# helgeanl/GP-MPC

Measured on NVIDIA H100. Metric: GP predictions/sec (N train x horizon test, fp64), higher is better.
Workload: dtype f64

## Files before the change

gp-mpc_b200/csrc/gpmpc.cu:

```cuda
#include "../../include/gpmpc.h"

#include <dlfcn.h>
#include <math.h>
#include <stdarg.h>
#include <stdlib.h>
#include <string.h>

#include <algorithm>
#include <array>
#include <functional>
#include <map>
#include <memory>
#include <type_traits>
#include <vector>

#include <nvtx3/nvToolsExt.h>

#include "common.cuh"
#include "gemm_dmma.cuh"
#include "predict_streamk.cuh"
#include "kernels.cuh"

#define GPMPC_VERSION 100
#define HB 64
// ... 1060 lines not shown
    if (!strcmp(name, "nlml_batch_max")) {
        if (!(value >= 0.0 && value <= 1e9)) { set_error(h, "nlml_batch_max must be >= 0"); return GPMPC_ERR_ARG; }
        h->opt_nlml_batch_max = (int)value; return GPMPC_OK;
    }
    set_error(h, "unknown option %s", name);
    return GPMPC_ERR_ARG;
}

static inline int ks_chunk(gpmpc_handle_t h)
{
    if (h->Npad < 8192) return 128;
    return (h->nloc >= 2 && h->Nx <= 12) ? 1024 : 512;
}

static inline int ks_blocks(gpmpc_handle_t h) { return (h->Npad + ks_chunk(h) - 1) / ks_chunk(h); }

static inline int round8(int n) { return (n + 7) / 8 * 8; }

static int ensure_rows(gpmpc_handle_t h)
{
    ENSURE(h->dV, (long long)h->nloc * HB * h->Npad);
    ENSURE(h->dR, (long long)h->nloc * HB * h->Npad);
    return GPMPC_OK;
}

static int ensure_predict_bufs(gpmpc_handle_t h, int H)
{
    const long long np = h->Npad, nt = np / 128;
    ENSURE(h->dKST, (long long)h->nloc * HB * np);
    ENSURE(h->dPMJ, (long long)h->nloc * HB * ks_blocks(h) * (h->Nx + 1));
    ENSURE(h->dSQ, (long long)h->nloc * HB * nt);
    ENSURE(h->dCnt, (long long)h->nloc * nt + h->nloc + 1);
    ENSURE(h->dPart, (long long)std::max(h->psk_ctas, h->opt_predict_ctas) * 2 * HB * PSK_BN);
    if (h->opt_refine) {
        int rc = ensure_rows(h);
        if (rc) return rc;
        ENSURE(h->dR2, (long long)h->nloc * HB * np);
    }
    if (H > h->Hcap) {
        h->Hcap = 0;
        h->dZ = h->dSigma = h->dMean = h->dVar = h->dJ = h->dCov = nullptr;
        const long long cap = std::max(H, HB);
        const int nyp = h->nloc_max * h->world;
        const long long Nx = h->Nx, Ny = h->Ny;
        ENSURE(h->dG, (long long)nyp * cap * (Nx + 2));
        ENSURE(h->dIn, cap * Nx + cap * Nx * Nx);
        ENSURE(h->dOut, cap * (2 * Ny + Ny * Nx + Ny * Ny));
        h->dZ = h->dIn; h->dSigma = h->dIn + cap * Nx;
        h->dMean = h->dOut; h->dVar = h->dOut + cap * Ny; h->dJ = h->dOut + 2 * cap * Ny;
        h->dCov = h->dOut + 2 * cap * Ny + cap * Ny * Nx;
        h->Hcap = (int)cap;
    }
    return GPMPC_OK;
}

template <int BM>
static cudaError_t psk_launch_bm(const PredictParams& p, const double* A, long long sA, const double* B, long long sB,
                                 int np, int grid, cudaStream_t st)
{
    constexpr int BYTES = psk_pipe_doubles(BM) * 8 + 2 * PSK_STAGES * 8 + 1024;
    const cudaError_t e = smem_opt_in<predict_streamk_kernel<BM>>(BYTES);
    if (e != cudaSuccess) return e;
    CUtensorMap tmA, tmB;
    if (!tmap_make(&tmA, A, np, BM, np, sA, p.nloc, BM)) return cudaErrorInvalidValue;
    if (!tmap_make(&tmB, B, np, np, np, sB, p.nloc, PSK_BN)) return cudaErrorInvalidValue;
    cudaLaunchConfig_t cfg;
    memset(&cfg, 0, sizeof(cfg));
    cfg.gridDim = dim3(grid); cfg.blockDim = dim3(PSK_THREADS); cfg.dynamicSmemBytes = BYTES; cfg.stream = st;
    cudaLaunchAttribute attr[1];
    attr[0].id = cudaLaunchAttributeProgrammaticStreamSerialization;
    attr[0].val.programmaticStreamSerializationAllowed = 1;
    cfg.attrs = attr; cfg.numAttrs = 1;
    return cudaLaunchKernelEx(&cfg, predict_streamk_kernel<BM>, p, tmA, tmB);
}

static int psk_grid(gpmpc_handle_t h, long long G)
{
    int ctas = h->opt_predict_ctas > 0 ? h->opt_predict_ctas : h->psk_ctas;
    ctas = std::min(ctas, PSK_MAX_CTAS);
    const long long by_work = std::max(1LL, G / 4);
    return (int)std::min<long long>(ctas, h->opt_predict_ctas > 0 ? G : by_work);
}

static cudaError_t psk_launch(gpmpc_handle_t h, const PredictParams& p0, const double* A, const double* B)
{
    const long long sA = (long long)HB * h->Npad, sB = slab(h);
    const int np = h->Npad, grid = psk_grid(h, p0.G);
    PredictParams p = p0;
    if (B == h->dLi.p && !p.upper) {
        for (int a = 0; a < h->nloc; ++a)
            if (h->panel_row[a] < np) return cudaErrorIllegalState;
        p.Lp = h->dLiP;
    }
    switch (round8(p.Hc)) {
    case 8: return psk_launch_bm<8>(p, A, sA, B, sB, np, grid, h->st);
    case 16: return psk_launch_bm<16>(p, A, sA, B, sB, np, grid, h->st);
    case 24: return psk_launch_bm<24>(p, A, sA, B, sB, np, grid, h->st);
    case 32: return psk_launch_bm<32>(p, A, sA, B, sB, np, grid, h->st);
    case 40: return psk_launch_bm<40>(p, A, sA, B, sB, np, grid, h->st);
    case 48: return psk_launch_bm<48>(p, A, sA, B, sB, np, grid, h->st);
    case 56: return psk_launch_bm<56>(p, A, sA, B, sB, np, grid, h->st);
    default: return psk_launch_bm<64>(p, A, sA, B, sB, np, grid, h->st);
    }
}

static void psk_base(gpmpc_handle_t h, PredictParams& p, int Hc, int upper = 0)
{
    memset(&p, 0, sizeof(p));
    const long long nt = h->Npad / 128;
    p.nloc = h->nloc; p.nt = (int)nt; p.Hc = Hc; p.upper = upper;
    p.ntb = (int)((h->Npad + PSK_BN - 1) / PSK_BN); p.nk = h->Npad / GEMM_BK;
    p.T = psk_steps_per_output(p.ntb, p.nk, upper); p.G = p.T * h->nloc;
    p.part = h->dPart;
    p.tile_cnt = h->dCnt; p.out_cnt = h->dCnt + (long long)h->nloc * nt; p.done_cnt = p.out_cnt + h->nloc;
    p.SQ = h->dSQ;
    p.hyp = h->dHyp; p.hyp_ld = h->Nx + 2; p.Nx = h->Nx;
}

static int panel_refresh(gpmpc_handle_t h)
{
    PredictParams p;
    psk_base(h, p, HB);
    const long long blk = PSK_BN * GEMM_BK;
    const double* old = h->dLiP;
    ENSURE(h->dLiP, p.G * blk);
    if (h->dLiP.p != old) panel_stale(h, -1, 0);
    for (int a = 0; a < h->nloc; ++a) {
        if (h->panel_row[a] >= h->Npad) continue;
        const int jt0 = h->panel_row[a] / PSK_BN;
        panel_pack_kernel<<<dim3(p.nk, p.ntb - jt0), 256, 0, h->st>>>(h->dLi + a * slab(h), h->Npad, h->dLiP + a * p.T * blk,
                                                                      p.ntb, jt0);
        CUDA_TRY(cudaGetLastError());
        h->panel_row[a] = h->Npad;
    }
    return GPMPC_OK;
}

static void psk_finalize(gpmpc_handle_t h, PredictParams& p, int H, int h0)
{
    p.finalize = 1; p.PMJ = h->dPMJ; p.nblk_mj = ks_blocks(h);
    p.Gloc = h->dG; p.slot0 = h->a0; p.Htot = H; p.h0 = h0;
}

static AssembleArgs assemble_args(gpmpc_handle_t h, int H, int method, const double* Sigma, int spp,
                                  double* mean, double* var, double* J, double* cov)
{
    AssembleArgs as;
    memset(&as, 0, sizeof(as));
    as.G = h->dG; as.Ny = h->Ny; as.Nx = h->Nx; as.H = H; as.method_ta = (method == GPMPC_METHOD_TA);
    as.Sigma = Sigma; as.sigma_per_point = spp;
    as.mean = mean; as.var = var; as.J = J; as.cov = cov;
    as.world = 1;
    as.stage_g = (assemble_rows_doubles(H, h->Ny, h->Nx) <= psk_pipe_doubles(round8(std::min(H, HB)))) ? 1 : 0;
    return as;
}

template <int NXP, int CH>
static cudaError_t launch_ks(gpmpc_handle_t h, const double* dZc, int Hc)
{
    const int smem = (NXP + 1) * CH * 8, nblk = ks_blocks(h);
    const cudaError_t e = smem_opt_in<ks_tile_kernel<NXP, CH>>(smem);
    if (e != cudaSuccess) return e;
    dim3 g(nblk, round8(Hc) / 8, h->nloc);
    ks_tile_kernel<NXP, CH><<<g, 256, smem, h->st>>>(h->dXT, h->Npad, h->N, h->Nx, h->dHyp, h->Nx + 2, h->dAlpha, h->Npad,
                                                     dZc, Hc, h->dKST, h->Npad, (long long)HB * h->Npad, h->dPMJ, nblk);
    return cudaGetLastError();
}

template <int CH>
static cudaError_t launch_ks_nx(gpmpc_handle_t h, const double* dZc, int Hc)
{
    const int Nx = h->Nx;
    if (Nx <= 4) return launch_ks<4, CH>(h, dZc, Hc);
    if (Nx <= 6) return launch_ks<6, CH>(h, dZc, Hc);
    if (Nx <= 8) return launch_ks<8, CH>(h, dZc, Hc);
    if (Nx <= 10) return launch_ks<10, CH>(h, dZc, Hc);
// ... 1658 lines not shown
    }
    if (world > 1) {
        if (!nccl_load(h->err, sizeof(h->err))) return GPMPC_ERR_NCCL;
        nccl_uid_t id;
        memcpy(&id, id128, 128);
        int r = g_nccl.CommInitRank(&h->comm, world, id, rank);
        if (r) { set_error(h, "ncclCommInitRank failed: %s", g_nccl.GetErrorString ? g_nccl.GetErrorString(r) : "?"); return GPMPC_ERR_NCCL; }
    }
    h->rank = rank; h->world = world; h->nloc_max = nlm;
    h->Hcap = 0;
    return GPMPC_OK;
}

extern "C" int gpmpc_peer_export(gpmpc_handle_t h, int Hcap, void* handle64)
{
    if (!h || !handle64 || Hcap < 1) return GPMPC_ERR_ARG;
    CUDA_TRY(cudaSetDevice(h->device));
    if (h->world > GPMPC_MAXW) { set_error(h, "peer exchange supports at most %d ranks", GPMPC_MAXW); return GPMPC_ERR_ARG; }
    if (h->dPeerBlock) { set_error(h, "gpmpc_peer_export: already exported"); return GPMPC_ERR_STATE; }
    const int nyp = h->nloc_max * h->world;
    h->peerGsz = (long long)nyp * Hcap * (h->Nx + 2);
    h->peerHcap = Hcap;
    ENSURE(h->dPeerBlock, 2 * GPMPC_MAXW + 2 * h->peerGsz);
    if (!h->dPeerStatus) {
        CUDA_TRY(cudaHostAlloc((void**)&h->hPeerStatus, sizeof(int), cudaHostAllocMapped));
        *h->hPeerStatus = 0;
        CUDA_TRY(cudaHostGetDevicePointer((void**)&h->dPeerStatus, h->hPeerStatus, 0));
    }
    CUDA_TRY(cudaStreamSynchronize(h->st));
    cudaIpcMemHandle_t mh;
    CUDA_TRY(cudaIpcGetMemHandle(&mh, h->dPeerBlock));
    static_assert(sizeof(cudaIpcMemHandle_t) == 64, "IPC handle size");
    memcpy(handle64, &mh, 64);
    return GPMPC_OK;
}

extern "C" int gpmpc_peer_attach(gpmpc_handle_t h, const void* handles)
{
    if (!h || !handles) return GPMPC_ERR_ARG;
    if (!h->dPeerBlock) { set_error(h, "gpmpc_peer_attach: call gpmpc_peer_export first"); return GPMPC_ERR_STATE; }
    CUDA_TRY(cudaSetDevice(h->device));
    for (int r = 0; r < h->world; ++r) {
        if (r == h->rank) { h->peerBase[r] = h->dPeerBlock; continue; }
        cudaIpcMemHandle_t mh;
        memcpy(&mh, (const char*)handles + 64 * r, 64);
        void* ptr = nullptr;
        CUDA_TRY(cudaIpcOpenMemHandle(&ptr, mh, cudaIpcMemLazyEnablePeerAccess));
        h->peerBase[r] = (double*)ptr; h->peerOpened[r] = true;
    }
    h->peer_ready = true; h->peer_step = 0;
    return GPMPC_OK;
}

extern "C" int gpmpc_get_size(gpmpc_handle_t h, int* N, int* Nx, int* Ny)
{
    if (!h) return GPMPC_ERR_ARG;
    if (N) *N = h->N;
    if (Nx) *Nx = h->Nx;
    if (Ny) *Ny = h->Ny;
    return GPMPC_OK;
}

extern "C" void* gpmpc_stream(gpmpc_handle_t h) { return h ? (void*)h->st : nullptr; }

extern "C" int gpmpc_synchronize(gpmpc_handle_t h)
{
    if (!h) return GPMPC_ERR_ARG;
    CUDA_TRY(cudaSetDevice(h->device));
    CUDA_TRY(cudaStreamSynchronize(h->st));
    return peer_status_check(h);
}

template <typename Setup>
static int profile_product(gpmpc_handle_t h, const char* fn, int H, const double* out, bool all_outputs, int n_tail,
                           Setup&& setup, std::vector<unsigned long long>& t, int* grid)
{
    if (!h || !out || H < 1 || H > HB) return GPMPC_ERR_ARG;
    int rc = predict_guard(h, fn, GPMPC_METHOD_TA, H);
    if (rc) return rc;
    rc = predict_prepare(h, fn, HB, all_outputs);
    if (rc) return rc;
    PredictParams p;
    psk_base(h, p, H);
    *grid = psk_grid(h, p.G);
    DevBuf<unsigned long long> dbg;
    ENSURE(dbg, (long long)*grid * 2 + n_tail);
    p.dbg = dbg;
    setup(p, dbg + 2 * *grid);
    for (int rep = 0; rep < 2; ++rep) {
        const cudaError_t e = psk_launch(h, p, h->dKST, h->dLi);
        if (e != cudaSuccess) { set_error(h, "%s: %s", fn, cudaGetErrorString(e)); return GPMPC_ERR_CUDA; }
    }
    t.resize((size_t)*grid * 2 + n_tail);
    cudaMemcpyAsync(t.data(), dbg, t.size() * 8, cudaMemcpyDeviceToHost, h->st);
    cudaStreamSynchronize(h->st);
    return GPMPC_OK;
}

extern "C" int gpmpc_profile_balance(gpmpc_handle_t h, int H, double* out4)
{
    std::vector<unsigned long long> t; int grid = 0;
    const int rc = profile_product(h, __func__, H, out4, false, 0, [](PredictParams&, unsigned long long*) {}, t, &grid);
    if (rc) return rc;
    unsigned long long lo = ~0ull, hi = 0; double mn = 1e300, mx = 0.0, sum = 0.0;
    for (int c = 0; c < grid; ++c) {
        const double d = (double)(t[2 * c + 1] - t[2 * c]) * 1e-3;
        mn = std::min(mn, d); mx = std::max(mx, d); sum += d;
        lo = std::min(lo, t[2 * c]); hi = std::max(hi, t[2 * c + 1]);
    }
    out4[0] = mn; out4[1] = mx; out4[2] = sum / grid; out4[3] = (double)(hi - lo) * 1e-3;
    return GPMPC_OK;
}

extern "C" int gpmpc_profile_tail(gpmpc_handle_t h, int H, double* out8)
{
    std::vector<unsigned long long> t; int grid = 0;
    auto setup = [&](PredictParams& p, unsigned long long* tail) {
        psk_finalize(h, p, H, 0);
        p.as = assemble_args(h, H, GPMPC_METHOD_TA, h->dSigma, 0, h->dMean, h->dVar, h->dJ, h->dCov);
        p.as.dbg = tail;
        p.do_assemble = 1;
    };
    const int rc = profile_product(h, __func__, H, out8, true, 8, setup, t, &grid);
    if (rc) return rc;
    unsigned long long lo = ~0ull, hi = 0, hi2 = 0; int cmax = 0;
    for (int c = 0; c < grid; ++c) {
        lo = std::min(lo, t[2 * c]);
        if (t[2 * c + 1] > hi) { hi2 = hi; hi = t[2 * c + 1]; cmax = c; } else hi2 = std::max(hi2, t[2 * c + 1]);
    }
    for (int k = 0; k < 6; ++k) out8[k] = ((double)t[2 * grid + k] - (double)hi2) * 1e-3;
    out8[6] = (double)(hi - lo) * 1e-3;
    out8[7] = (double)(t[2 * cmax + 1] - t[2 * cmax]) * 1e-3;
    return GPMPC_OK;
}

extern "C" int gpmpc_profile_leaf(gpmpc_handle_t h, double* out15)
{
    if (!h || !out15) return GPMPC_ERR_ARG;
    int rc = model_guard(h, __func__, NEED_HYPER);
    if (rc) return rc;
    DevBuf<long long> d;
    ENSURE(d, 16);
    CUDA_TRY(cudaMemcpyToSymbol(d_leaf_prof, &d.p, sizeof(d.p)));
    for (int rep = 0; rep < 2 && rc == GPMPC_OK; ++rep) {
        rc = launch_kbuild(h, h->dHyp, h->dJit, h->dL, 1, 0);
        if (rc == GPMPC_OK) rc = potrf_inv_rec(h, h->dL, h->dLi, slab(h), slab(h), h->dInfo, 0, 128, 1, 1, h->dW1, h->dW2);
    }
    cudaStreamSynchronize(h->st);
    long long hst[16];
    cudaMemcpy(hst, d, sizeof(hst), cudaMemcpyDeviceToHost);
    long long* nul = nullptr;
    cudaMemcpyToSymbol(d_leaf_prof, &nul, sizeof(nul));
    for (int k = 0; k < 15; ++k) out15[k] = (double)(hst[k] - hst[0]);
    factor_stale(h);
    return rc;
}

extern "C" int gpmpc_profile(gpmpc_handle_t h, int what, int n, int reps, double* ms_out)
{
    if (!h || !ms_out || reps < 1) return GPMPC_ERR_ARG;
    int rc = model_guard(h, __func__, NEED_HYPER);
    if (rc) return rc;
    const int np = h->Npad, Hc = (n > 0 && n <= HB) ? n : 56;
    float ms = 0.f;
    auto run = [&]() -> int {
        switch (what) {
        case GPMPC_PROF_KBUILD_FULL: return launch_kbuild(h, h->dHyp, h->dJit, h->dL, 1, 1);
// ... 62 lines not shown
```

gp-mpc_b200/csrc/predict_streamk.cuh:

```cuda
#pragma once
#include "common.cuh"
#include "gemm_dmma.cuh"

#define GPMPC_MAXW 16
#define PSK_CW 8
#define PSK_BN (32 * PSK_CW)
#define PSK_STAGES 5
#define PSK_CTAS_PER_SM 1
#define PSK_THREADS (32 * PSK_CW)

__host__ __device__ constexpr long long psk_pipe_doubles(int bm) { return (long long)PSK_STAGES * (bm + PSK_BN) * GEMM_BK; }


struct PeerArgs {
    double* base[GPMPC_MAXW];
    int world, rank;
    long long goff;
    int flag_idx;
    unsigned long long step;
    long long timeout_clocks;
};

struct AssembleArgs {
    const double* G;
    int Ny, Nx, H, method_ta;
    const double* Sigma; int sigma_per_point;
    double *mean, *var, *J, *cov;
    const unsigned long long* flags;
    int world; unsigned long long step; int* status;
    long long timeout_clocks;
    unsigned long long* dbg;
    int stage_g;
};

struct PredictParams {
    int nloc, nt, Hc;
    int ntb, nk;
    int upper;
    const double* Lp;
    long long T, G;
    double* part;
    unsigned int* tile_cnt;
    unsigned int* out_cnt;
    unsigned int* done_cnt;
    double* SQ;
    double* Vout; long long sV; int ldv;
    int finalize;
    const double* PMJ; int nblk_mj;
    const double* hyp; int hyp_ld, Nx;
    double* Gloc; int slot0, Htot, h0;
    PeerArgs pa; int use_peers, publish;
    AssembleArgs as; int do_assemble;
    unsigned long long* dbg;
};

__device__ __forceinline__ void tail_stamp(unsigned long long* dbg, int k, int tid)
{
    if (dbg && tid == 0) { unsigned long long t; asm volatile("mov.u64 %0, %%globaltimer;" : "=l"(t)); dbg[k] = t; }
}

template <bool WARP>
__device__ __forceinline__ void assemble_point(const AssembleArgs& A, int h, double* sh, int tid, int nth)
{
    const int Ny = A.Ny, Nx = A.Nx, H = A.H;
    double* Jh = sh; double* JS = sh + Ny * Nx; double* vh = sh + 2 * Ny * Nx;
    for (int idx = tid; idx < Ny * Nx; idx += nth) {
        const int a = idx / Nx, d = idx % Nx;
        const double v = __ldcg(A.G + (((long long)a) * H + h) * (Nx + 2) + 2 + d);
        Jh[idx] = v;
        if (A.J) A.J[((long long)h * Ny + a) * Nx + d] = v;
    }
    for (int a = tid; a < Ny; a += nth) {
        const double* g = A.G + (((long long)a) * H + h) * (Nx + 2);
        const double m = __ldcg(g), v = __ldcg(g + 1);
        if (A.mean) A.mean[(long long)h * Ny + a] = m;
        if (A.var) A.var[(long long)h * Ny + a] = v;
        vh[a] = v;
    }
    if (WARP) __syncwarp(); else __syncthreads();
    if (A.cov) {
        if (A.method_ta) {
            const double* Sg = A.Sigma + (A.sigma_per_point ? (long long)h * Nx * Nx : 0);
            for (int idx = tid; idx < Ny * Nx; idx += nth) {
                const int a = idx / Nx, e = idx % Nx;
                double s = 0.0;
                for (int d = 0; d < Nx; ++d) s = fma(Jh[a * Nx + d], Sg[d * Nx + e], s);
                JS[idx] = s;
            }
            if (WARP) __syncwarp(); else __syncthreads();
        }
        for (int idx = tid; idx < Ny * Ny; idx += nth) {
            const int a = idx / Ny, b = idx % Ny;
            double s = (a == b) ? vh[a] : 0.0;
            if (A.method_ta) {
                double t = 0.0;
                for (int e = 0; e < Nx; ++e) t = fma(JS[a * Nx + e], Jh[b * Nx + e], t);
                s += t;
            }
            A.cov[((long long)h * Ny + a) * Ny + b] = s;
        }
    }
    if (WARP) __syncwarp(); else __syncthreads();
}

__device__ __forceinline__ void assemble_flat_global(const AssembleArgs& A, double* JS, int tid, int nth)
{
    const int Ny = A.Ny, Nx = A.Nx, H = A.H, NyNx = Ny * Nx;
    const bool ta = A.cov && A.method_ta;
    for (int idx = tid; idx < H * NyNx; idx += nth) {
        const int h = idx / NyNx, r = idx - h * NyNx, a = r / Nx, e = r - a * Nx;
        const double* g = A.G + (((long long)a) * H + h) * (Nx + 2) + 2;
        if (A.J) A.J[idx] = __ldcg(g + e);
        if (ta) {
            const double* Sg = A.Sigma + (A.sigma_per_point ? (long long)h * Nx * Nx : 0);
            double s = 0.0;
            for (int d = 0; d < Nx; ++d) s = fma(__ldcg(g + d), Sg[d * Nx + e], s);
            JS[idx] = s;
        }
    }
    for (int idx = tid; idx < H * Ny; idx += nth) {
        const int h = idx / Ny, a = idx - h * Ny;
        const double* g = A.G + (((long long)a) * H + h) * (Nx + 2);
        if (A.mean) A.mean[idx] = __ldcg(g);
// ... 77 lines not shown
        const bool via_smem = Ny <= 8 && Ny <= NP;
        for (int idx = tid; idx < R; idx += nth) {
            const int h = idx / Ny, a = idx - h * Ny;
            const double var = Gs[idx * FP + 1];
            for (int b0 = 0; b0 < Ny; b0 += 8) {
                double acc[8];
#pragma unroll
                for (int k = 0; k < 8; ++k) acc[k] = 0.0;
                if (ta) {
                    for (int e = 0; e < Nx; ++e) {
                        const double je = JS[idx * NP + e];
#pragma unroll
                        for (int k = 0; k < 8; ++k) if (b0 + k < Ny) acc[k] = fma(je, Gs[(h * Ny + b0 + k) * FP + 2 + e], acc[k]);
                    }
                }
#pragma unroll
                for (int k = 0; k < 8; ++k) {
                    if (b0 + k < Ny) {
                        const double c = ((a == b0 + k) ? var : 0.0) + acc[k];
                        if (via_smem) JS[idx * NP + k] = c; else A.cov[(long long)idx * Ny + b0 + k] = c;
                    }
                }
            }
        }
        if (via_smem) {
            __syncthreads();
            for (int i = tid; i < R * Ny; i += nth) { const int row = i / Ny; A.cov[i] = JS[row * NP + (i - row * Ny)]; }
        }
    }
}

__device__ __forceinline__ void assemble_flat(const AssembleArgs& A, double* sh, int tid, int nth)
{
    if (A.stage_g) assemble_rows(A, sh, tid, nth);
    else assemble_flat_global(A, sh, tid, nth);
}

__device__ __forceinline__ bool peer_acquire(const AssembleArgs& A, int tid, int* sh_ok)
{
    if (!A.flags) return true;
    if (tid == 0) *sh_ok = 1;
    __syncthreads();
    if (tid < A.world) {
        const long long t0 = clock64();
        unsigned long long v;
        do {
            asm volatile("ld.acquire.sys.global.u64 %0, [%1];" : "=l"(v) : "l"(A.flags + tid) : "memory");
            if (v >= A.step) break;
            if (clock64() - t0 > A.timeout_clocks) {
                *reinterpret_cast<volatile int*>(A.status) = 1 + tid;
                *reinterpret_cast<volatile int*>(sh_ok) = 0;
                break;
            }
            __nanosleep(64);
        } while (true);
    }
    __syncthreads();
    return *reinterpret_cast<volatile int*>(sh_ok) != 0;
}

__global__ void __launch_bounds__(128)
assemble_kernel(const AssembleArgs A)
{
    extern __shared__ double sh[];
    __shared__ int ok;
    if (!peer_acquire(A, threadIdx.x, &ok)) return;
    for (int h = blockIdx.x; h < A.H; h += gridDim.x) assemble_point<false>(A, h, sh, threadIdx.x, blockDim.x);
}

#define PSK_SB (PSK_BN / GEMM_BK)
__host__ __device__ inline long long psk_kstart(int ntb, int nk, int upper, int jt)
{
    const long long full = (long long)(PSK_SB / 2) * jt * (jt + 1), d = (long long)PSK_SB * ntb - nk;
    return upper ? full - jt * d : (jt == ntb ? full - d : full);
}
__host__ __device__ inline long long psk_steps_per_output(int ntb, int nk, int upper) { return psk_kstart(ntb, nk, upper, ntb); }
__device__ __forceinline__ long long psk_kstart(const PredictParams& p, int jt) { return psk_kstart(p.ntb, p.nk, p.upper, jt); }
__host__ __device__ inline int psk_ksteps(int ntb, int nk, int upper, int jt)
{
    return upper ? nk - PSK_SB * (ntb - 1 - jt) : (PSK_SB * (jt + 1) < nk ? PSK_SB * (jt + 1) : nk);
}
__device__ __forceinline__ int psk_ksteps(const PredictParams& p, int jt) { return psk_ksteps(p.ntb, p.nk, p.upper, jt); }

struct PskIter { int a, jt, s, ks; };

__device__ __forceinline__ void psk_iter_init(PskIter& it, long long g, const PredictParams& p)
{
    it.a = (int)(g / p.T);
    const long long r = g - (long long)it.a * p.T;
    int jt = (int)((sqrt(8.0 * (double)r / PSK_SB + 1.0) - 1.0) * 0.5);
    jt = max(0, min(jt, p.ntb - 1));
    while (jt > 0 && psk_kstart(p, jt) > r) --jt;
    while (jt + 1 < p.ntb && psk_kstart(p, jt + 1) <= r) ++jt;
    it.jt = jt; it.s = (int)(r - psk_kstart(p, jt)); it.ks = psk_ksteps(p, jt);
}
__device__ __forceinline__ void psk_iter_next(PskIter& it, const PredictParams& p)
{
    if (++it.s == it.ks) {
        it.s = 0;
        if (++it.jt == p.ntb) { it.jt = 0; ++it.a; }
        it.ks = psk_ksteps(p, it.jt);
    }
}

__host__ __device__ inline long long psk_panel_chunk(int ntb, int nk, int jt, int s, int r, int c)
{
    return (psk_kstart(ntb, nk, 0, jt) + s) * (PSK_BN * GEMM_BK) + r * GEMM_BK + 2 * (c ^ (r & 7));
}

__global__ void __launch_bounds__(256)
panel_pack_kernel(const double* __restrict__ Li, int np, double* __restrict__ P, int ntb, int jt0)
{
    const int s = blockIdx.x, jt = jt0 + blockIdx.y, nk = np / GEMM_BK, c = threadIdx.x & 7;
    if (s >= psk_ksteps(ntb, nk, 0, jt)) return;
#pragma unroll 4
    for (int r = threadIdx.x >> 3; r < PSK_BN; r += 32) {
        const long long row = (long long)jt * PSK_BN + r;
        const double2 v = row < np ? __ldcs(reinterpret_cast<const double2*>(Li + row * np + s * GEMM_BK) + c) : make_double2(0.0, 0.0);
        *reinterpret_cast<double2*>(P + psk_panel_chunk(ntb, nk, jt, s, r, c)) = v;
    }
}

__device__ __forceinline__ void psk_store_record(const PredictParams& p, int a, int h, int q, double val)
{
    const long long off = (((long long)(p.slot0 + a)) * p.Htot + p.h0 + h) * (p.Nx + 2) + q;
    if (!p.use_peers) p.Gloc[off] = val;
    else for (int r = 0; r < p.pa.world; ++r) p.pa.base[r][p.pa.goff + off] = val;
}

__device__ __forceinline__ void psk_reduce_mj(const PredictParams& p, int i_begin, int i_end, int t, int nthr)
{
    const int F1 = p.Nx + 1;
    for (int i = i_begin + t; i < i_end; i += nthr) {
        const int ah = i / F1, qq = i - ah * F1, a = ah / p.Hc, h = ah - a * p.Hc;
        const double* pm = p.PMJ + ((long long)ah * p.nblk_mj) * F1 + qq;
        double s0 = 0.0, s1 = 0.0;
        int b = 0;
        for (; b + 16 <= p.nblk_mj; b += 16) {
            double v[16];
#pragma unroll
            for (int k = 0; k < 16; ++k) v[k] = __ldcg(pm + (long long)(b + k) * F1);
#pragma unroll
            for (int k = 0; k < 16; k += 2) { s0 += v[k]; s1 += v[k + 1]; }
        }
        for (; b + 2 <= p.nblk_mj; b += 2) { s0 += __ldcg(pm + (long long)b * F1); s1 += __ldcg(pm + (long long)(b + 1) * F1); }
        if (b < p.nblk_mj) s0 += __ldcg(pm + (long long)b * F1);
        psk_store_record(p, a, h, qq == 0 ? 0 : qq + 1, s0 + s1);
    }
}

__device__ __forceinline__ void psk_finalize_output(const PredictParams& p, int a, int tid, int nth)
{
    const int Nx = p.Nx;
    const double sf = p.hyp[(long long)a * p.hyp_ld + Nx];
    for (int base = 0; base < p.Hc; base += nth / 4) {
        const int h = base + (tid >> 2), j0 = tid & 3;
        double sj = 0.0;
        if (h < p.Hc) {
            const double* sq = p.SQ + ((long long)a * 64 + h) * p.nt;
            int j = j0;
            for (; j + 4 * 15 < p.nt; j += 4 * 16) {
                double v[16];
#pragma unroll
                for (int k = 0; k < 16; ++k) v[k] = __ldcg(sq + j + 4 * k);
#pragma unroll
                for (int k = 0; k < 16; ++k) sj += v[k];
            }
            for (; j < p.nt; j += 4) sj += __ldcg(sq + j);
        }
        sj += __shfl_xor_sync(0xffffffffu, sj, 1);
        sj += __shfl_xor_sync(0xffffffffu, sj, 2);
        if (h < p.Hc && j0 == 0) psk_store_record(p, a, h, 1, sf * sf - sj);
    }
    if (p.use_peers) __threadfence_system(); else __threadfence();
}

__device__ __forceinline__ void psk_step_tail(const PredictParams& p, double* sh, int tid, int nth,
                                              unsigned int* s_flag, int* s_ok)
{
    __syncthreads();
    if (tid == 0) {
        const unsigned int old = atomicAdd(p.done_cnt, 1u);
        const unsigned int last = (old == (unsigned int)(p.nloc - 1)) ? 1u : 0u;
        if (last) *p.done_cnt = 0u;
        *s_flag = last;
    }
    __syncthreads();
    if (*s_flag == 0u) return;
    if (p.finalize && p.use_peers && p.publish && tid == 0) {
        __threadfence_system();
        for (int r = 0; r < p.pa.world; ++r) {
            unsigned long long* f = reinterpret_cast<unsigned long long*>(p.pa.base[r]) + p.pa.flag_idx;
            asm volatile("st.release.sys.global.u64 [%0], %1;" :: "l"(f), "l"(p.pa.step) : "memory");
        }
    }
    tail_stamp(p.as.dbg, 2, tid);
    if (p.do_assemble) {
        __threadfence();
        if (peer_acquire(p.as, tid, s_ok)) assemble_flat(p.as, sh, tid, nth);
    }
    __syncthreads();
    tail_stamp(p.as.dbg, 5, tid);
}

__global__ void __launch_bounds__(128)
sq_rows_kernel(const double* __restrict__ V, int ldv, long long sV, double* __restrict__ SQ, int nt)
{
    __shared__ double red[4];
    const int jt = blockIdx.x, h = blockIdx.y, a = blockIdx.z;
    const double v = V[(long long)a * sV + (long long)h * ldv + jt * 128 + threadIdx.x];
    const double s = warp_sum(v * v);
    if ((threadIdx.x & 31) == 0) red[threadIdx.x >> 5] = s;
    __syncthreads();
    if (threadIdx.x == 0) SQ[((long long)a * 64 + h) * nt + jt] = (red[0] + red[1]) + (red[2] + red[3]);
}

__global__ void __launch_bounds__(PSK_THREADS)
finalize_kernel(const PredictParams p)
{
    extern __shared__ double sh[];
    __shared__ unsigned int s_flag;
    __shared__ int s_ok;
    const int per = p.Hc * (p.Nx + 1);
    psk_reduce_mj(p, blockIdx.x * per, (blockIdx.x + 1) * per, threadIdx.x, PSK_THREADS);
    psk_finalize_output(p, blockIdx.x, threadIdx.x, PSK_THREADS);
    psk_step_tail(p, sh, threadIdx.x, PSK_THREADS, &s_flag, &s_ok);
}

template <int BM>
__global__ void __launch_bounds__(PSK_THREADS, PSK_CTAS_PER_SM)
predict_streamk_kernel(const PredictParams p, const __grid_constant__ CUtensorMap tmA, const __grid_constant__ CUtensorMap tmB)
{
    constexpr int BK = GEMM_BK, BN = PSK_BN, STAGES = PSK_STAGES, CW = PSK_CW, NT = PSK_THREADS;
    constexpr int NF = BM / 8;
    static_assert(BK == 16 && BN == 32 * CW && BN % 128 == 0, "one m16n8k16 per fragment and k-step, 32 L-rows per warp");
    constexpr int GR = BN / 128;
    constexpr int A_STAGE = BM * BK, B_STAGE = BN * BK;
    constexpr uint32_t STAGE_TX = (BM + BN) * BK * 8;
    static_assert(BM % 8 == 0 && BM >= 8 && BM <= 64, "BM");

    extern __shared__ __align__(16) double smem_raw[];
    double* smem = smem_align1024(smem_raw);
    double* As = smem;
    double* Bs = smem + STAGES * A_STAGE;
    uint64_t* full = reinterpret_cast<uint64_t*>(smem + STAGES * (A_STAGE + B_STAGE));
    uint64_t* empty = full + STAGES;
    __shared__ double red[BN / 16][64];
    __shared__ unsigned int s_flag;
    __shared__ int s_ok;

    const int tid = threadIdx.x, warp = tid >> 5, lane = tid & 31, g = lane >> 2, t = lane & 3;
    const long long C = gridDim.x, c = blockIdx.x;
    const long long g0 = p.G * c / C;
    const int nsteps = (int)(p.G * (c + 1) / C - g0);
    if (nsteps <= 0) return;
    if (p.dbg && threadIdx.x == 0) { unsigned long long t0; asm volatile("mov.u64 %0, %%globaltimer;" : "=l"(t0)); p.dbg[2 * blockIdx.x] = t0; }

    __shared__ PskIter s_pit;
    __shared__ int s_pg;
    __shared__ uint64_t s_pol[2];
    __shared__ const double* s_lp;
    if (tid == 0) {
#pragma unroll
        for (int s = 0; s < STAGES; ++s) { mbar_init(full + s, 1); mbar_init(empty + s, CW); }
        mbar_fence_init();
    }
    __syncthreads();

    auto issue = [&]() {
        PskIter it = s_pit;
        const int pg = s_pg, s = pg % STAGES;
        if (pg >= STAGES) mbar_wait(empty + s, (uint32_t)(((pg / STAGES) - 1) & 1));
        mbar_arrive_expect_tx(full + s, STAGE_TX);
        const int jta = p.upper ? p.ntb - 1 - it.jt : it.jt;
        const int k0 = (p.upper ? jta * BN : 0) + it.s * BK;
        tma_tile_g2s_3d_hint(As + s * A_STAGE, &tmA, k0, 0, it.a, full + s, s_pol[1]);
        if (s_lp) bulk_g2s_hint(Bs + s * B_STAGE, s_lp + (long long)pg * B_STAGE, B_STAGE * 8, full + s, s_pol[0]);
        else tma_tile_g2s_3d_hint(Bs + s * B_STAGE, &tmB, k0, jta * BN, it.a, full + s, s_pol[0]);
        psk_iter_next(it, p);
        s_pit = it;
        s_pg = pg + 1;
    };
    constexpr int AHEAD = STAGES - 2;
    asm volatile("griddepcontrol.wait;" ::: "memory");
    if (tid == 0) {
        PskIter it;
        psk_iter_init(it, g0, p);
        s_pit = it; s_pg = 0;
        s_lp = p.Lp ? p.Lp + g0 * B_STAGE : nullptr;
        s_pol[0] = l2_policy_evict_first(); s_pol[1] = l2_policy_evict_last();
#pragma unroll
        for (int s = 0; s < AHEAD; ++s)
            if (s_pg < nsteps) issue();
    }
    if (p.finalize) {
        const int tot = p.nloc * p.Hc * (p.Nx + 1), per = (tot + (int)C - 1) / (int)C;
        if (tid >= 32) {
            psk_reduce_mj(p, min(tot, (int)c * per), min(tot, ((int)c + 1) * per), tid - 32, NT - 32);
            if (p.use_peers) __threadfence_system();
        }
    }

    PskIter cit;
    psk_iter_init(cit, g0, p);
    int cj[4];
#pragma unroll
    for (int j = 0; j < 4; ++j) cj[j] = (((j + 4 * (t >> 1)) ^ g) << 1) + (t & 1);
    int i = 0;
    while (i < nsteps) {
        const int a = cit.a, jt = cit.jt, s_begin = cit.s, ksteps = cit.ks;
        const int seg = min(ksteps - s_begin, nsteps - i);
        const int hh = warp / (128 / 32);
        const int st_lo = p.upper ? (128 / BK) * hh : 0;
        const int st_hi = p.upper ? ksteps : PSK_SB * jt + (128 / BK) * (hh + 1);
        double acc[2][NF][4];
#pragma unroll
        for (int mi = 0; mi < 2; ++mi)
#pragma unroll
            for (int ni = 0; ni < NF; ++ni)
#pragma unroll
                for (int r = 0; r < 4; ++r) acc[mi][ni][r] = 0.0;

        for (int q = 0; q < seg; ++q, ++i) {
            const int s = i % STAGES;
            if (tid == 0 && i + AHEAD < nsteps) issue();
            mbar_wait(full + s, (uint32_t)((i / STAGES) & 1));
            const int st = s_begin + q;
            if (st >= st_lo && st < st_hi) {
                const double* ls = Bs + s * B_STAGE + (warp * 32 + g) * 16;
                const double* ps = As + s * A_STAGE + g * 16;
                double av[2][8];
#pragma unroll
                for (int mi = 0; mi < 2; ++mi)
#pragma unroll
                    for (int j = 0; j < 4; ++j) { av[mi][2 * j] = ls[256 * mi + cj[j]]; av[mi][2 * j + 1] = ls[256 * mi + 128 + cj[j]]; }
#pragma unroll
                for (int ni = 0; ni < NF; ++ni) {
                    double bv[4];
#pragma unroll
                    for (int j = 0; j < 4; ++j) bv[j] = ps[ni * 8 * 16 + cj[j]];
                    dmma16816(acc[0][ni], av[0], bv);
                    dmma16816(acc[1][ni], av[1], bv);
                }
            }
            __syncwarp();
            if (lane == 0) mbar_arrive(empty + s);
        }
        cit.s = s_begin + seg - 1;
        psk_iter_next(cit, p);

        bool have_tile = true;
        if (seg != ksteps) {
            const long long tg0 = (long long)a * p.T + psk_kstart(p, jt), tg1 = tg0 + ksteps;
            const long long Cf = gridDim.x;
            const int c_first = (int)(((tg0 + 1) * Cf - 1) / p.G), c_last = (int)((tg1 * Cf - 1) / p.G);
            double2* mine = reinterpret_cast<double2*>(p.part + ((long long)blockIdx.x * 2 + (s_begin == 0 ? 1 : 0)) * (BM * BN)) + tid;
#pragma unroll
            for (int mi = 0; mi < 2; ++mi)
#pragma unroll
                for (int ni = 0; ni < NF; ++ni)
#pragma unroll
                    for (int hf = 0; hf < 2; ++hf)
                        __stcg(mine + ((mi * NF + ni) * 2 + hf) * NT, make_double2(acc[mi][ni][2 * hf], acc[mi][ni][2 * hf + 1]));
            __threadfence();
            __syncthreads();
            if (tid == 0) {
                unsigned int* cnt = p.tile_cnt + (long long)a * p.ntb + jt;
                const unsigned int old = atomicAdd(cnt, 1u);
                const unsigned int last = (old == (unsigned int)(c_last - c_first)) ? 1u : 0u;
                if (last) *cnt = 0u;
                s_flag = last;
            }
            __syncthreads();
            have_tile = s_flag != 0u;
            if (have_tile) {
                __threadfence();
#pragma unroll
                for (int mi = 0; mi < 2; ++mi)
#pragma unroll
                    for (int ni = 0; ni < NF; ++ni)
#pragma unroll
                        for (int r = 0; r < 4; ++r) acc[mi][ni][r] = 0.0;
                for (int cc = c_first; cc <= c_last; ++cc) {
                    const double2* src = reinterpret_cast<const double2*>(p.part + ((long long)cc * 2 + (cc == c_first ? 1 : 0)) * (BM * BN)) + tid;
#pragma unroll
                    for (int mi = 0; mi < 2; ++mi)
#pragma unroll
// ... 67 lines not shown
```

Measured before the change: 15180.

## Schedule stream-K predict work as paired triangular tile units per CTA

New measurement: 16600 (median of 6 runs). 9.4% higher.

```diff
diff --git a/gp-mpc_b200/csrc/gpmpc.cu b/gp-mpc_b200/csrc/gpmpc.cu
--- a/gp-mpc_b200/csrc/gpmpc.cu
+++ b/gp-mpc_b200/csrc/gpmpc.cu
@@ -1166,16 +1166,26 @@
     return (int)std::min<long long>(ctas, h->opt_predict_ctas > 0 ? G : by_work);
 }
 
+static int psk_schedule(gpmpc_handle_t h, PredictParams& p, const double* B)
+{
+    int grid = psk_grid(h, p.G);
+    if (B == h->dLi.p && !p.upper) {
+        p.Lp = h->dLiP;
+        p.upo = psk_pair_units(p.nloc, p.ntb, grid);
+        if (p.upo && h->opt_predict_ctas == 0) grid = psk_pair_grid((long long)p.nloc * p.upo, grid);
+    }
+    return grid;
+}
+
 static cudaError_t psk_launch(gpmpc_handle_t h, const PredictParams& p0, const double* A, const double* B)
 {
     const long long sA = (long long)HB * h->Npad, sB = slab(h);
-    const int np = h->Npad, grid = psk_grid(h, p0.G);
+    const int np = h->Npad;
     PredictParams p = p0;
-    if (B == h->dLi.p && !p.upper) {
+    const int grid = psk_schedule(h, p, B);
+    if (p.Lp)
         for (int a = 0; a < h->nloc; ++a)
             if (h->panel_row[a] < np) return cudaErrorIllegalState;
-        p.Lp = h->dLiP;
-    }
     switch (round8(p.Hc)) {
     case 8: return psk_launch_bm<8>(p, A, sA, B, sB, np, grid, h->st);
     case 16: return psk_launch_bm<16>(p, A, sA, B, sB, np, grid, h->st);
@@ -3000,7 +3010,7 @@
     if (rc) return rc;
     PredictParams p;
     psk_base(h, p, H);
-    *grid = psk_grid(h, p.G);
+    *grid = psk_schedule(h, p, h->dLi);
     DevBuf<unsigned long long> dbg;
     ENSURE(dbg, (long long)*grid * 2 + n_tail);
     p.dbg = dbg;
diff --git a/gp-mpc_b200/csrc/predict_streamk.cuh b/gp-mpc_b200/csrc/predict_streamk.cuh
--- a/gp-mpc_b200/csrc/predict_streamk.cuh
+++ b/gp-mpc_b200/csrc/predict_streamk.cuh
@@ -39,6 +39,7 @@
     int upper;
     const double* Lp;
     long long T, G;
+    int upo;
     double* part;
     unsigned int* tile_cnt;
     unsigned int* out_cnt;
@@ -282,10 +283,48 @@
 }
 __device__ __forceinline__ int psk_ksteps(const PredictParams& p, int jt) { return psk_ksteps(p.ntb, p.nk, p.upper, jt); }
 
+__host__ __device__ inline int psk_pair_units(int nloc, int ntb, int grid)
+{
+    const long long upo = (ntb + 1) / 2, units = nloc * upo, rounds = (units + grid - 1) / grid;
+    return (units >= grid && 8 * units >= 7 * rounds * grid) ? (int)upo : 0;
+}
+__host__ __device__ inline int psk_pair_grid(long long units, int grid)
+{
+    const long long rounds = (units + grid - 1) / grid;
+    return (int)((units + rounds - 1) / rounds);
+}
+__host__ __device__ inline int psk_unit_steps(int ntb, int nk, int pu)
+{
+    const int jl = ntb - 1 - pu;
+    return psk_ksteps(ntb, nk, 0, jl) + (pu != jl ? psk_ksteps(ntb, nk, 0, pu) : 0);
+}
+__host__ __device__ inline long long psk_pair_cta_steps(int nloc, int ntb, int nk, int upo, long long c, long long C)
+{
+    long long n = 0;
+    for (long long u = c; u < (long long)nloc * upo; u += C) n += psk_unit_steps(ntb, nk, (int)(u % upo));
+    return n;
+}
+__host__ __device__ inline void psk_pair_first(int ntb, int upo, long long u, int& a, int& jt)
+{
+    a = (int)(u / upo);
+    jt = ntb - 1 - (int)(u - (long long)a * upo);
+}
+__host__ __device__ inline void psk_pair_next(int ntb, int upo, long long C, int& a, int& jt)
+{
+    if (2 * jt > ntb - 1) jt = ntb - 1 - jt;
+    else psk_pair_first(ntb, upo, (long long)a * upo + jt + C, a, jt);
+}
+
 struct PskIter { int a, jt, s, ks; };
 
-__device__ __forceinline__ void psk_iter_init(PskIter& it, long long g, const PredictParams& p)
-{
+__device__ __forceinline__ void psk_iter_init(PskIter& it, const PredictParams& p, long long c, long long C)
+{
+    if (p.upo) {
+        psk_pair_first(p.ntb, p.upo, c, it.a, it.jt);
+        it.s = 0; it.ks = psk_ksteps(p, it.jt);
+        return;
+    }
+    const long long g = p.G * c / C;
     it.a = (int)(g / p.T);
     const long long r = g - (long long)it.a * p.T;
     int jt = (int)((sqrt(8.0 * (double)r / PSK_SB + 1.0) - 1.0) * 0.5);
@@ -298,7 +337,8 @@
 {
     if (++it.s == it.ks) {
         it.s = 0;
-        if (++it.jt == p.ntb) { it.jt = 0; ++it.a; }
+        if (p.upo) psk_pair_next(p.ntb, p.upo, gridDim.x, it.a, it.jt);
+        else if (++it.jt == p.ntb) { it.jt = 0; ++it.a; }
         it.ks = psk_ksteps(p, it.jt);
     }
 }
@@ -451,15 +491,14 @@
 
     const int tid = threadIdx.x, warp = tid >> 5, lane = tid & 31, g = lane >> 2, t = lane & 3;
     const long long C = gridDim.x, c = blockIdx.x;
-    const long long g0 = p.G * c / C;
-    const int nsteps = (int)(p.G * (c + 1) / C - g0);
+    const int nsteps = p.upo ? (int)psk_pair_cta_steps(p.nloc, p.ntb, p.nk, p.upo, c, C)
+                             : (int)(p.G * (c + 1) / C - p.G * c / C);
     if (nsteps <= 0) return;
     if (p.dbg && threadIdx.x == 0) { unsigned long long t0; asm volatile("mov.u64 %0, %%globaltimer;" : "=l"(t0)); p.dbg[2 * blockIdx.x] = t0; }
 
     __shared__ PskIter s_pit;
     __shared__ int s_pg;
     __shared__ uint64_t s_pol[2];
-    __shared__ const double* s_lp;
     if (tid == 0) {
 #pragma unroll
         for (int s = 0; s < STAGES; ++s) { mbar_init(full + s, 1); mbar_init(empty + s, CW); }
@@ -475,7 +514,8 @@
         const int jta = p.upper ? p.ntb - 1 - it.jt : it.jt;
         const int k0 = (p.upper ? jta * BN : 0) + it.s * BK;
         tma_tile_g2s_3d_hint(As + s * A_STAGE, &tmA, k0, 0, it.a, full + s, s_pol[1]);
-        if (s_lp) bulk_g2s_hint(Bs + s * B_STAGE, s_lp + (long long)pg * B_STAGE, B_STAGE * 8, full + s, s_pol[0]);
+        if (p.Lp) bulk_g2s_hint(Bs + s * B_STAGE, p.Lp + ((long long)it.a * p.T + psk_kstart(p, it.jt) + it.s) * B_STAGE,
+                                B_STAGE * 8, full + s, s_pol[0]);
         else tma_tile_g2s_3d_hint(Bs + s * B_STAGE, &tmB, k0, jta * BN, it.a, full + s, s_pol[0]);
         psk_iter_next(it, p);
         s_pit = it;
@@ -485,9 +525,8 @@
     asm volatile("griddepcontrol.wait;" ::: "memory");
     if (tid == 0) {
         PskIter it;
-        psk_iter_init(it, g0, p);
+        psk_iter_init(it, p, c, C);
         s_pit = it; s_pg = 0;
-        s_lp = p.Lp ? p.Lp + g0 * B_STAGE : nullptr;
         s_pol[0] = l2_policy_evict_first(); s_pol[1] = l2_policy_evict_last();
 #pragma unroll
         for (int s = 0; s < AHEAD; ++s)
@@ -502,7 +541,7 @@
     }
 
     PskIter cit;
-    psk_iter_init(cit, g0, p);
+    psk_iter_init(cit, p, c, C);
     int cj[4];
 #pragma unroll
     for (int j = 0; j < 4; ++j) cj[j] = (((j + 4 * (t >> 1)) ^ g) << 1) + (t & 1);
```
